# Strong-AI-Lab/ct-vae

Hardware: AMD Instinct MI355X
Metric: images/sec/GPU fwd+bwd, 64×64×3 bs=64; recon+KL vs CPU ref (higher is better)
Workload: dtype f32; 1 GPU; VanillaVAE 64x64x3 train step fwd+loss+bwd+Adam (configs/vae.yaml shapes at the batch BASELINE.json's metric names, bs=64, on one MI355X; BASELINE.json configs[1..4] are the `configs` entries); per_gpu_batch=64, global_batch=64, latent_dim=128, parallelism=single, hipgraph=True, allreduce_overlap=False

## Files before the change

ct-vae_amd/csrc/api.hip:

```cpp
#include "../../include/ctvae_hip.h"

#include "common.hpp"
#include "gatlayer.hpp"
#include "glinear.hpp"
#include "pair.hpp"

namespace ctvae {
int launch_tapgemm(const ConvGeom& g, const float* G, const float* W, const float* bias, const float* add,
                   const float* mask, int mask_act, float* S, int act, float* bn_part, float* ws, size_t ws_floats,
                   hipStream_t st, const BnBwdFuse* bnb = nullptr, const InXform* xf = nullptr,
                   const WinoFilters* wf = nullptr, SplitKRaw* raw = nullptr, int out_pix = 0);
bool out_pix_supported(const ConvGeom& g, size_t ws_floats, int out_pix);
bool wino_supported(const ConvGeom& g, size_t ws_floats);
bool wino_enabled();
int wino_set_enabled(int on);
int launch_crop_resize_u8(const unsigned char* img, const long long* rows, float* out, int B, int N, int H, int W, int crop,
                          int S, hipStream_t st);
bool thin_forward_supported(const ConvGeom& g);
bool thin_wgrad_supported(const ConvGeom& g);
int tapgemm_bnb_rows(const ConvGeom& g, size_t ws_floats);
bool img_dgrad_supported(const ConvGeom& g);
void tapgemm_plan(const ConvGeom& g, size_t ws_floats, TapGemmPlan& p);
int launch_wgrad(const ConvGeom& g, const float* X, const float* dY, float* dW, float* dbias, float* ws, size_t ws_bytes,
                 int accumulate, hipStream_t st, const InXform* xf = nullptr, const DyXform* dyx = nullptr);
int launch_bn_forward(const float* y, int R, int C, const float* gamma, const float* beta, float* running_mean,
                      float* running_var, float momentum, float eps, int training, int act, float* out, float* save_mean,
                      float* save_invstd, float* ws, size_t ws_bytes, long long* nbt, hipStream_t st,
                      float* coef_out = nullptr);
int launch_bn_finish_forward(const float* y, int R, int C, int nparts, const float* gamma, const float* beta,
                             float* running_mean, float* running_var, float momentum, float eps, int training, int act,
                             float* out, float* save_mean, float* save_invstd, float* ws, long long* nbt, hipStream_t st,
                             float* coef_out = nullptr);
size_t bn_workspace_floats(int C, int nparts);
int launch_bn_backward(const float* ga, const float* beta, const float* y, int R, int C, const float* gamma,
                       const float* save_mean, const float* save_invstd, int act, float* gy, float* dgamma, float* dbeta,
                       int accumulate, float* ws, size_t ws_bytes, const float* part_in, int part_rows, hipStream_t st,
                       float* coef_out = nullptr, const float* coef_in = nullptr);
int launch_wino_filters_batch(int n, const float* const* W, float* const* Uf, float* const* Ub, const int* Ci, const int* Co,
                              hipStream_t st);
bool upconv_wgrad_supported(const ConvGeom& g);
bool img_enc_supported(const ConvGeom& g);
bool img_conv_supported(const ConvGeom& g);
int launch_img_backward_fused(const ConvGeom& g, const float* dY, const float* W, float* dX, const BnBwdFuse* bnb, float* ws,
                              float** part_out, float** pbias_out, int* nparts, bool want_bias, hipStream_t st);
size_t img_backward_fused_ws_floats(const ConvGeom& g);
int wgrad_finish_slabs(const float* part, float* dW, long n, int nparts, const float* pbias, float* dbias, long nb, int accumulate,
                       hipStream_t st);
int launch_permute(const float* in, float* out, int B, int C, int P, int to_nhwc, hipStream_t st);
int launch_gat_score(int mode, const float* xl, const float* xr, const float* attr, const float* we, const float* att, float* out,
                     int B, int N, int H, int C, float slope, hipStream_t st);
int launch_gat_score_backward(const float* xl, const float* xr, const float* attr, const float* we, const float* att,
                              const float* g, float* dxl, float* dxr, float* datt_part, float* dwe_part, int B, int N, int H,
                              int C, float slope, hipStream_t st);
int launch_gauss_latent_fwd(float* heads, const float* eps_in, const unsigned long long* rng, float* eps_out, float* z, int B,
                            int L, hipStream_t st, const float* slices, int S, const float* bias);
int launch_splitk_permute(const float* slices, int S, float* out, int B, int C, int P, hipStream_t st);
int launch_gauss_latent_bwd(const float* g_mu, const float* g_lv, const float* g_z, const float* heads, const float* eps,
                            float* g_heads, unsigned long long* rng_bump, int B, int L, hipStream_t st, int gz_slices);
int launch_ct_reg_forward(const float* adj, const float* graph, const float* uni, float* part, float ckl, float cgs, float cpt,
                          int B, int N, hipStream_t st);
int launch_ct_reg_backward(const float* adj, const float* graph, const float* uni, const float* part, const float* g_loss,
                           float ckl, float cgs, float cpt, float* d_adj, float* d_graph, int B, int N, hipStream_t st);
int launch_ct_blend_softmax_forward(const float* y, const float* mask, float* probs, long R, int Hs, int D, hipStream_t st);
int launch_ct_blend_softmax_backward(const float* g, const float* probs, const float* y, const float* mask, float* dy, float* dmask,
                                     long R, int Hs, int D, hipStream_t st);
int launch_ct_latent_ce_forward(const float* probs, const long long* target, float* row_loss, long R, int D, hipStream_t st);
int launch_ct_latent_ce_backward(const float* probs, const long long* target, const float* g_loss, float* d_probs, long R, int D,
                                 hipStream_t st);
int launch_ct_mask_forward(const float* x, const float* action, const float* pe, const float* keep, float scale, const float* W,
                           const float* bias, const float* expo, int B, int S, int D, int A, float* inter, float* p, float* sample,
// ... 440 lines not shown
}

int ctvae_conv_wgrad_bn_apply_supported(int kind, int B, int H, int W, int Ci, int Co, int k, int stride, int pad, int out_pad) {
  if (!conv_kind_ok(kind)) return 0;
  ConvGeom g;
  if (conv_geom(g, kind, 0, B, H, W, Ci, Co, k, stride, pad, out_pad)) return 0;
  if (upconv_wgrad_supported(g)) return 1;
  return img_enc_supported(g) ? 2 : 0;
}

int ctvae_bn_forward(const float* y, int R, int C, const float* gamma, const float* beta, float* running_mean,
                     float* running_var, float momentum, float eps, int training, int act, float* out,
                     float* save_mean, float* save_invstd, int64_t* num_batches_tracked, float* ws, size_t ws_bytes,
                     void* stream) {
  if (!y || !gamma || !beta || !out || !ws) return kErrBadArg;
  if (training && (!save_mean || !save_invstd)) return kErrBadArg;
  if (!training && (!running_mean || !running_var)) return kErrBadArg;
  return launch_bn_forward(y, R, C, gamma, beta, running_mean, running_var, momentum, eps, training, act, out, save_mean,
                           save_invstd, ws, ws_bytes, (long long*)num_batches_tracked, (hipStream_t)stream);
}

int ctvae_bn_backward(const float* g_a, const float* beta, const float* y, int R, int C, const float* gamma,
                      const float* save_mean, const float* save_invstd, int act, float* g_y, float* dgamma,
                      float* dbeta, int accumulate, const float* part_in, int part_rows, float* coef_out,
                      const float* coef_in, float* ws, size_t ws_bytes, void* stream) {
  if (!g_a || !beta || !y || !gamma || !save_mean || !save_invstd || !dgamma || !dbeta || !ws) return kErrBadArg;
  if (!g_y && !coef_out) return kErrBadArg;
  if ((part_in != nullptr) != (part_rows > 0)) return kErrBadArg;
  if (coef_in != nullptr && (!g_y || part_in != nullptr || coef_out != nullptr)) return kErrBadArg;
  return launch_bn_backward(g_a, beta, y, R, C, gamma, save_mean, save_invstd, act, g_y, dgamma, dbeta, accumulate, ws,
                            ws_bytes, part_in, part_rows, (hipStream_t)stream, coef_out, coef_in);
}

int ctvae_gat_score(int mode, const float* xl, const float* xr, const float* attr, const float* we, const float* att, float* out,
                    int B, int N, int H, int C, float slope, void* stream) {
  if (!xl || !xr || !attr || !we || !att || !out || (mode != 0 && mode != 1)) return kErrBadArg;
  return launch_gat_score(mode, xl, xr, attr, we, att, out, B, N, H, C, slope, (hipStream_t)stream);
}

int ctvae_gat_score_backward(const float* xl, const float* xr, const float* attr, const float* we, const float* att,
                             const float* g, float* d_xl, float* d_xr, float* d_att_part, float* d_we_part, int B, int N, int H,
                             int C, float slope, void* stream) {
  if (!xl || !xr || !attr || !we || !att || !g || !d_xl || !d_xr || !d_att_part || !d_we_part) return kErrBadArg;
  return launch_gat_score_backward(xl, xr, attr, we, att, g, d_xl, d_xr, d_att_part, d_we_part, B, N, H, C, slope,
                                   (hipStream_t)stream);
}

int ctvae_gat_layer_forward(const float* xl, const float* xr, int ld, const float* adj, const float* we, const float* att,
                            const float* bias, const int32_t* head_map, float* out, int ldo, float* alpha, int B, int Hs, int C,
                            float slope, int act, void* stream) {
  const GatLayerArgs a{xl, xr, ld, adj, we, att, bias, head_map, out, ldo, alpha, B, Hs, C, slope, act};
  return launch_gat_layer_forward(a, (hipStream_t)stream);
}

int ctvae_gat_layer_backward(const float* xl, const float* xr, int ld, const float* adj, const float* we, const float* att,
                             const float* bias, const int32_t* head_map, const float* out, int ldo, const float* alpha,
                             const float* g_out, float* dS, float* dattr, float* d_xl, float* d_xr, int ldd, float* d_bias_part,
                             float* d_att_part, float* d_we_part, float* d_adj, int accumulate_dadj, int B, int Hs, int C,
                             float slope, int act, void* stream) {
  GatBwdArgs p{};
  p.f = GatLayerArgs{xl, xr, ld, adj, we, att, bias, head_map, const_cast<float*>(out), ldo, const_cast<float*>(alpha), B, Hs, C,
                     slope, act};
  p.g_out = g_out; p.dS = dS; p.dattr = dattr; p.dxl = d_xl; p.dxr = d_xr; p.ldd = ldd;
  p.dbias_part = d_bias_part; p.datt_part = d_att_part; p.dwe_part = d_we_part;
  return launch_gat_layer_backward(p, d_adj, accumulate_dadj, (hipStream_t)stream);
}
// ... 473 lines not shown
```

ct-vae_amd/csrc/bn.hip:

```cpp
#include "common.hpp"
#include "phase.hpp"
#include "finish.hpp"
#include "prof.hpp"

namespace ctvae {
__device__ __forceinline__ float act_dt(float t, int act, float slope) {
  return act == ACT_TANH ? act_bwd_from_out(act_fwd(t, ACT_TANH), ACT_TANH) : act_slope_bwd(t, slope);
}


constexpr int kBnMaxBlocks = 2048;

__device__ __forceinline__ void chan_merge(float& n, float& mean, float& m2, float nb, float mb, float qb) {
  if (nb > 0.f) {
    const float nt = n + nb, d = mb - mean;
    mean += d * (nb / nt);
    m2 += qb + d * d * (n * nb / nt);
    n = nt;
  }
}

__global__ __launch_bounds__(256) void bn_stats_partial_kernel(const float* __restrict__ y, float* __restrict__ part,
                                                               int R, int C, int rows_per_block) {
  __shared__ float sm[256 * 9];
// ... 315 lines not shown
  }
  s1 = wave_sum_d(s1);
  s2 = wave_sum_d(s2);
  if ((tid & 63) == 0) { sm[(tid >> 6) * 2] = s1; sm[(tid >> 6) * 2 + 1] = s2; }
  __syncthreads();
  if (tid == 0) {
    s1 = (sm[0] + sm[2]) + (sm[4] + sm[6]);
    s2 = (sm[1] + sm[3]) + (sm[5] + sm[7]);
    const float db = (float)s1, dg = (float)s2;
    dgamma[c] = (accumulate ? dgamma[c] : 0.f) + dg;
    dbeta[c] = (accumulate ? dbeta[c] : 0.f) + db;
    const float invstd = save_invstd[c], mean = save_mean[c];
    const float k1 = gamma[c] * invstd;
    const float k2 = -k1 * dg / R * invstd;
    const float k3 = -k1 * db / R - k2 * mean;
    coef[c] = k1;
    coef[C + c] = k2;
    coef[2 * C + c] = k3;
    coef[3 * C + c] = k1;
    coef[4 * C + c] = beta[c] - mean * k1;
  }
}

__global__ __launch_bounds__(256) void bn_bwd_finalize_apply_kernel(const float* __restrict__ ga, const float* __restrict__ y,
                                                                    const float* __restrict__ part, int nblocks, int R, int C,
                                                                    const float* __restrict__ gamma, const float* __restrict__ save_mean,
                                                                    const float* __restrict__ save_invstd, const float* __restrict__ beta,
                                                                    int act, float* __restrict__ gy, float* __restrict__ dgamma,
                                                                    float* __restrict__ dbeta, int accumulate) {
  __shared__ double smd[256 * 2];
  __shared__ __attribute__((aligned(16))) float sK[5][32];
  const int tid = threadIdx.x, cb = blockIdx.x, rs = blockIdx.y;
  const int c0 = cb * 32, ch = tid & 31, rl = tid >> 5;
  double s1 = 0.0, s2 = 0.0;
  for (int b = rl; b < nblocks; b += 8) {
    s1 += (double)part[((long)b * C + c0 + ch) * 2 + 0];
    s2 += (double)part[((long)b * C + c0 + ch) * 2 + 1];
  }
  smd[tid * 2] = s1; smd[tid * 2 + 1] = s2;
  __syncthreads();
  if (rl == 0) {
    for (int l = 1; l < 8; ++l) {
      s1 += smd[(l * 32 + ch) * 2];
      s2 += smd[(l * 32 + ch) * 2 + 1];
    }
    const int c = c0 + ch;
    const float db = (float)s1, dg = (float)s2;
    const float invstd = save_invstd[c], mean = save_mean[c];
    const float k1 = gamma[c] * invstd;
    const float k2 = -k1 * dg / (float)R * invstd;
    const float k3 = -k1 * db / (float)R - k2 * mean;
    sK[0][ch] = k1; sK[1][ch] = k2; sK[2][ch] = k3; sK[3][ch] = k1; sK[4][ch] = beta[c] - mean * k1;
    if (rs == 0) {
      dgamma[c] = (accumulate ? dgamma[c] : 0.f) + dg;
      dbeta[c] = (accumulate ? dbeta[c] : 0.f) + db;
    }
  }
  __syncthreads();
  const int q = tid & 7;
  const f32x4 k1 = *reinterpret_cast<const f32x4*>(&sK[0][4 * q]), k2 = *reinterpret_cast<const f32x4*>(&sK[1][4 * q]);
  const f32x4 k3 = *reinterpret_cast<const f32x4*>(&sK[2][4 * q]), sc = *reinterpret_cast<const f32x4*>(&sK[3][4 * q]);
  const f32x4 sh = *reinterpret_cast<const f32x4*>(&sK[4][4 * q]);
  const int rows_per = (R + gridDim.y - 1) / gridDim.y;
  const int r0 = rs * rows_per, r1 = r0 + rows_per < R ? r0 + rows_per : R;
  for (int r = r0 + (tid >> 3); r < r1; r += 32) {
    const long i = ((long)r * C + c0) / 4 + q;
    const f32x4 g = reinterpret_cast<const f32x4*>(ga)[i], yv = reinterpret_cast<const f32x4*>(y)[i];
    f32x4 o;
#pragma unroll
    for (int k = 0; k < 4; ++k)
      o[k] = k1[k] * (g[k] * act_dt(yv[k] * sc[k] + sh[k], act, act_slope(act))) + k2[k] * yv[k] + k3[k];
    reinterpret_cast<f32x4*>(gy)[i] = o;
  }
}

__global__ __launch_bounds__(256) void bn_bwd_finalize_job_kernel(BnFinJob j) {
  __shared__ double sm[8];
  bn_bwd_finalize_body(j, blockIdx.x, sm);
// ... 363 lines not shown
  } else {
    hipLaunchKernelGGL(bn_eval_coeff_kernel, dim3(ceil_div(C, 256)), dim3(256), 0, st, C, gamma, beta, running_mean,
                       running_var, eps, scale, shift);
    CTVAE_LAUNCH_CHECK();
  }
  if (out == nullptr) return 0;
  const long n4 = (long)R * C / 4;
  long blocks = (n4 + 255) / 256;
  if (blocks > 4096) blocks = 4096;
  ProfScope ps("bn_apply_act_kernel", st, 0.0, 8.0 * (double)R * C);
  hipLaunchKernelGGL(bn_apply_act_kernel, dim3((unsigned)blocks), dim3(256), 0, st, y, scale, shift, out, n4, C, act);
  CTVAE_LAUNCH_CHECK();
  return 0;
}

int launch_bn_forward(const float* y, int R, int C, const float* gamma, const float* beta, float* running_mean,
                      float* running_var, float momentum, float eps, int training, int act, float* out,
                      float* save_mean, float* save_invstd, float* ws, size_t ws_bytes, long long* nbt, hipStream_t st,
                      float* coef_out) {
  if (!bn_shape_ok(R, C)) return kErrBadArg;
  if (ws_bytes / sizeof(float) < bn_workspace_floats(C, 0)) return kErrWorkspace;
  int nb = 0;
  if (training) {
    int rpb;
    nb = stat_blocks(R, C, &rpb);
    ProfScope ps("bn_stats_partial_kernel", st, 0.0, 4.0 * (double)R * C);
    hipLaunchKernelGGL(bn_stats_partial_kernel, dim3(nb), dim3(256), 0, st, y, ws, R, C, rpb);
    CTVAE_LAUNCH_CHECK();
  }
  return launch_bn_finish_forward(y, R, C, nb, gamma, beta, running_mean, running_var, momentum, eps, training, act, out,
                                  save_mean, save_invstd, ws, nbt, st, coef_out);
}

int launch_bn_backward(const float* ga, const float* beta, const float* y, int R, int C, const float* gamma,
                       const float* save_mean, const float* save_invstd, int act, float* gy, float* dgamma,
                       float* dbeta, int accumulate, float* ws, size_t ws_bytes, const float* part_in, int part_rows,
                       hipStream_t st, float* coef_out, const float* coef_in) {
  if (!bn_shape_ok(R, C)) return kErrBadArg;
  if (coef_in != nullptr) {
    if (gy == nullptr) return kErrBadArg;
    ProfScope ps("bn_bwd_apply_kernel", st, 0.0, 12.0 * (double)R * C);
    const long n4 = (long)R * C / 4;
    long blocks = (n4 + 255) / 256;
    if (blocks > 4096) blocks = 4096;
    hipLaunchKernelGGL(bn_bwd_apply_kernel, dim3((unsigned)blocks), dim3(256), 0, st, ga, y, coef_in, gy, n4, C, act, dgamma,
                       dbeta, accumulate);
    CTVAE_LAUNCH_CHECK();
    return 0;
  }
  if (ws_bytes / sizeof(float) < bn_workspace_floats(C, 0)) return kErrWorkspace;
  const float* part = ws;
  float* coef = coef_out != nullptr ? coef_out : ws + (size_t)kBnMaxBlocks * C * 3;
  int rpb;
  int nb = stat_blocks(R, C, &rpb);
  if (part_in != nullptr && part_rows > 0) {
    part = part_in;
    nb = part_rows;
  } else {
    ProfScope ps("bn_bwd_partial_kernel", st, 0.0, 8.0 * (double)R * C);
    hipLaunchKernelGGL(bn_bwd_partial_kernel, dim3(nb), dim3(256), 0, st, ga, gamma, beta, y, save_mean, save_invstd, ws, R,
                       C, rpb, act);
  }
  CTVAE_LAUNCH_CHECK();
  if (part_in != nullptr && gy != nullptr && coef_out == nullptr && nb <= 256 && C % 32 == 0) {
    int rsn = 512 / (C / 32);
    if (rsn > R / 32) rsn = R / 32;
    if (rsn < 1) rsn = 1;
    ProfScope ps("bn_bwd_finalize_apply_kernel", st, 0.0, 12.0 * (double)R * C + 8.0 * (double)nb * C * rsn);
    hipLaunchKernelGGL(bn_bwd_finalize_apply_kernel, dim3(C / 32, rsn), dim3(256), 0, st, ga, y, part, nb, R, C, gamma, save_mean,
                       save_invstd, beta, act, gy, dgamma, dbeta, accumulate);
    CTVAE_LAUNCH_CHECK();
    return 0;
  }
  {
    ProfScope ps("bn_bwd_finalize_kernel", st, 0.0, 8.0 * (double)nb * C);
    hipLaunchKernelGGL(bn_bwd_finalize_kernel, dim3(C), dim3(256), 0, st, part, nb, C, (float)R, gamma,
                       save_mean, save_invstd, dgamma, dbeta, accumulate, beta, coef);
  }
  CTVAE_LAUNCH_CHECK();
  if (gy == nullptr) return 0;
  ProfScope ps("bn_bwd_apply_kernel", st, 0.0, 12.0 * (double)R * C);
  const long n4 = (long)R * C / 4;
  long blocks = (n4 + 255) / 256;
  if (blocks > 4096) blocks = 4096;
  hipLaunchKernelGGL(bn_bwd_apply_kernel, dim3((unsigned)blocks), dim3(256), 0, st, ga, y, coef, gy, n4, C, act, (float*)nullptr,
                     (float*)nullptr, 0);
  CTVAE_LAUNCH_CHECK();
  return 0;
}

int launch_bn_bwd_finalize_job(const BnFinJob& j, hipStream_t st) {
  ProfScope ps("bn_bwd_finalize_kernel", st, 0.0, 8.0 * (double)j.nblocks * j.C);
  hipLaunchKernelGGL(bn_bwd_finalize_job_kernel, dim3(j.C), dim3(256), 0, st, j);
  CTVAE_LAUNCH_CHECK();
  return 0;
}

// ... 2 lines not shown
```

ct-vae_amd/kernels.py:

```python
import math
import weakref
from dataclasses import dataclass

import torch
from torch.autograd import Function

from . import native

ACT_NONE, ACT_LRELU, ACT_RELU, ACT_TANH = 0, 1, 2, 3
CONV, CONVT = 0, 1
CONV_FLAT = CONV | 0x100
BN_MOMENTUM, BN_EPS = 0.1, 1e-5


@dataclass(frozen=True)
class ConvSpec:
    kind: int
    ci: int
    co: int
    k: int
    stride: int = 1
    pad: int = 0
    out_pad: int = 0
    act: int = ACT_NONE
# ... 124 lines not shown

def _wino_filters_for(ctx_needs_grad, w, spec, B, H, W_):
    n = wino_filter_floats(spec, B, H, W_, native.workspace(w.device).numel()) if ctx_needs_grad else 0
    if not n:
        return None, None
    if _WINO_BATCH and spec.ci % 32 == 0 and spec.co % 32 == 0:
        uf, ub = wino_cache.filters(w, spec, n)
        return uf, ub
    return None, torch.empty(n, dtype=torch.float32, device=w.device)


def conv_dgrad_raw(dy, w, spec: ConvSpec, in_hw, add=None, mask=None, mask_act=ACT_NONE, wino_filters=None):
    B = dy.shape[0]
    H, W = in_hw
    dx = torch.empty((B, H, W, spec.ci), dtype=torch.float32, device=dy.device)
    ws = native.workspace(dy.device)
    if wino_filters is not None and wino_filter_floats(spec, B, H, W, ws.numel()) != wino_filters.numel():
        wino_filters = None
    g = spec.geom(B, H, W)
    native.call("ctvae_conv_dgrad", g[0], dy.data_ptr(), w.data_ptr(), native.ptr(add), native.ptr(mask), mask_act,
                dx.data_ptr(), *g[1:], native.ptr(wino_filters), ws.data_ptr(), ws.numel() * 4)
    return dx


def _stamp(t):
    return t.data_ptr(), t._version, tuple(t.shape)


def _same(t, stamp):
    return stamp is not None and _stamp(t) == stamp


class BNLink:
    __slots__ = ("y", "mean", "invstd", "gamma", "beta", "act", "part", "rows", "coef", "g", "slices", "sole", "g_hold")

    def __init__(self, y, mean, invstd, gamma, beta, act):
        self.y, self.mean, self.invstd, self.gamma, self.beta, self.act = y, mean, invstd, gamma, beta, act
        self.sole = False
        self.g_hold = None
        self.part = None
        self.rows = 0
        self.coef = None
        self.slices = None
        self.g = None

    def publish_lazy(self, g, slices, n, geom):
        self.slices = (slices, n, geom)
        self.g_hold = g
        self.part, self.rows, self.coef = None, 0, None
        self.g = _stamp(g)

    def take_lazy(self, g):
        sl, self.slices = self.slices, None
        self.g_hold = None
        if sl is None:
            return None
        if not _same(g, self.g):
            raise RuntimeError("BNLink: the consumer left its data gradient as split-K slices for this BatchNorm's backward pass "
                               "(sole consumer of the layer's output), but a different gradient tensor arrived")
        return sl

    def publish(self, g, part, rows, coef=None):
        self.part, self.rows, self.coef = part, rows, coef
        self.g = _stamp(g)

    def take(self, g):
        part, rows, coef = self.part, self.rows, self.coef
        self.part, self.rows, self.coef = None, 0, None
        if part is None or not _same(g, self.g):
            return None, 0, None
        return part, rows, coef
# ... 80 lines not shown


def pop_lazy_bn():
    global _last_lazy
    lz, _last_lazy = _last_lazy, None
    return lz


def bn_apply_is_separate(spec, B, H, W) -> bool:
    ws = native.workspace(torch.device("cuda", torch.cuda.current_device()))
    return bool(_geom_query("ctvae_conv_bn_act_apply_is_separate", spec.geom(B, H, W), ws.numel() * 4))


def lazy_bn_input_supported(spec, B, H, W) -> bool:
    return input_transform_supported(spec, B, H, W)


def pop_bn_link():
    global _last_link
    link, _last_link = _last_link, None
    return link


def mark_sole_consumer(x):
    link = getattr(x, "_ctvae_bn_link", None)
    if link is not None:
        link.sole = True
    return x


def link_of(x):
    link = getattr(x, "_ctvae_bn_link", None)
    return link if (link is not None and x.is_contiguous()) else None


def _dy_bn_args(dy_bn):
    return (dy_bn[0].data_ptr(), dy_bn[1].data_ptr(), dy_bn[2], native.ptr(dy_bn[3])) if dy_bn is not None else (None, None, 0, None)


def _bn_commit_args(bn_commit):
    return (bn_commit[0].data_ptr(), bn_commit[1].data_ptr(), bn_commit[2]) if bn_commit is not None else (None, None, 0)


def conv_wgrad_raw(x, dy, w_param, b_param, spec: ConvSpec, in_coef=None, in_act=ACT_NONE, dy_bn=None, bn_commit=None):
    B, H, W, _ = x.shape
    ws = native.workspace(x.device)
    gw, gb, acc = _grad_targets(w_param, b_param)
    g = spec.geom(B, H, W)
    native.call("ctvae_conv_wgrad", g[0], x.data_ptr(), dy.data_ptr(), gw.data_ptr(), native.ptr(gb), *g[1:], acc,
                *_coef_ptrs(in_coef, spec.ci), in_act, *_dy_bn_args(dy_bn), *_bn_commit_args(bn_commit),
                ws.data_ptr(), ws.numel() * 4)


_PAIR = True


def _conv_backward_lazy(x, dy, w_param, gw, gb, acc, spec, in_coef, in_act, pixel_major):
    B, H, W, _ = x.shape
    ws = native.workspace(x.device)
    g = spec.geom(B, H, W)
    n = _geom_query("ctvae_conv_backward_lazy_slices", g, 0 if pixel_major else 1, ws.numel() * 4)
    if n <= 1:
        return None
    slices = torch.empty(n * B * H * W * spec.ci, dtype=torch.float32, device=dy.device)
    native.call("ctvae_conv_backward_lazy", g[0], x.data_ptr(), dy.data_ptr(), w_param.data_ptr(), gw.data_ptr(), native.ptr(gb),
                slices.data_ptr(), *g[1:], acc, *_coef_ptrs(in_coef, spec.ci), in_act, pixel_major, ws.data_ptr(), ws.numel() * 4)
    return slices, n


def conv_backward_raw(x, dy, w_param, b_param, spec: ConvSpec, link=None, mask=None, mask_act=ACT_NONE, wino_filters=None,
                      in_coef=None, in_act=ACT_NONE, dy_bn=None, bn_commit=None, grad_slices=False):
    B, H, W, _ = x.shape
    ws = native.workspace(x.device)
    g = spec.geom(B, H, W)
    if wino_filters is not None and wino_filter_floats(spec, B, H, W, ws.numel() // 2) != wino_filters.numel():
        wino_filters = None
    gw, gb, acc = _grad_targets(w_param, b_param)
    dx = torch.empty((B, H, W, spec.ci), dtype=torch.float32, device=dy.device)
    if (link is not None and link.sole and tuple(link.y.shape) == (B, H, W, spec.ci) and mask is None and wino_filters is None
            and dy_bn is None and bn_commit is None):
        lazy = _conv_backward_lazy(x, dy, w_param, gw, gb, acc, spec, in_coef, in_act, 0)
        if lazy is not None:
            link.publish_lazy(dx, *lazy, g)
            return dx
    if grad_slices and link is None and mask is None and wino_filters is None and dy_bn is None and bn_commit is None:
        lazy = _conv_backward_lazy(x, dy, w_param, gw, gb, acc, spec, in_coef, in_act, 1)
        if lazy is not None:
            offer_lazy_grad(dx, *lazy)
            return dx
    part, rows = None, 0
    if link is not None and tuple(link.y.shape) == (B, H, W, spec.ci):
        rows = max(_geom_query("ctvae_conv_backward_bn_rows", g, ws.numel() * 4), 0)
        if rows > 0:
            part = torch.empty(rows * spec.ci * 2, dtype=torch.float32, device=dy.device)
    bn = link if part is not None else None
    coef = torch.empty(7 * spec.ci, dtype=torch.float32, device=dy.device) if bn is not None else None
    cg, cb, cacc = _bn_commit_args(bn_commit)
    if coef is None:
        cg = cb = None
    native.call("ctvae_conv_backward", g[0], x.data_ptr(), dy.data_ptr(), w_param.data_ptr(), gw.data_ptr(), native.ptr(gb),
                dx.data_ptr(), *g[1:], acc, native.ptr(mask), mask_act, native.ptr(wino_filters),
                native.ptr(bn.y if bn else None), native.ptr(bn.mean if bn else None), native.ptr(bn.invstd if bn else None),
                native.ptr(bn.gamma if bn else None), native.ptr(bn.beta if bn else None), bn.act if bn else 0,
                native.ptr(part), rows, native.ptr(coef), cg, cb, cacc,
                *_coef_ptrs(in_coef, spec.ci), in_act, *_dy_bn_args(dy_bn), ws.data_ptr(), ws.numel() * 4)
    if bn is not None:
        bn.publish(dx, part, rows, coef)
    return dx


def wgrad_then_dgrad(x, g, w_param, b_param, spec, need_dgrad, link=None, wino_filters=None, in_coef=None, in_act=ACT_NONE,
                     grad_slices=False):
    if need_dgrad:
        return conv_backward_raw(x, g, w_param, b_param, spec, link=link, wino_filters=wino_filters, in_coef=in_coef, in_act=in_act,
                                 grad_slices=grad_slices)
    conv_wgrad_raw(x, g, w_param, b_param, spec, in_coef=in_coef, in_act=in_act)
    return None


def act_backward_raw(g_out, out, act):
    if act == ACT_NONE:
        return g_out
    g_in = torch.empty_like(out)
    native.call("ctvae_act_backward", g_out.data_ptr(), out.data_ptr(), g_in.data_ptr(), out.numel(), act)
    return g_in


def permute_raw(x, B, C, P, to_nhwc):
    out = torch.empty(x.numel(), dtype=torch.float32, device=x.device)
# ... 296 lines not shown
                *_coef_ptrs(in_coef, spec.ci), in_act, ws.data_ptr(), ws.numel() * 4)
    return y, a, coef, save_mean, save_invstd


def _bn_backward(g_a, y, bn, bn_act, g_y, grads, part=None, rows=0, coef_out=None, coef_in=None):
    gamma, beta, save_mean, save_invstd = bn
    gg, gbt, acc = grads
    B, H, W, C = y.shape
    ws = native.workspace(y.device)
    native.call("ctvae_bn_backward", g_a.data_ptr(), beta.data_ptr(), y.data_ptr(), B * H * W, C, gamma.data_ptr(),
                save_mean.data_ptr(), save_invstd.data_ptr(), bn_act, native.ptr(g_y), gg.data_ptr(), gbt.data_ptr(), acc,
                native.ptr(part), rows, native.ptr(coef_out), native.ptr(coef_in), ws.data_ptr(), ws.numel() * 4)


class ConvBNAct(Function):

    @staticmethod
    def forward(ctx, x, w, b, gamma, beta, running_mean, running_var, training, spec, bn_act, num_batches_tracked=None,
                lazy_out=False):
        global _last_link
        _req_cuda(x, w, gamma)
        ctx.link_in = link_of(x)
        ctx.x_slices_ok = bool(getattr(x, "_ctvae_grad_slices_ok", False))
        lazy_in = getattr(x, "_ctvae_lazy_bn", None) if x.is_contiguous() else None
        x = _c(x)
        y, a, coef, save_mean, save_invstd = _conv_bn_act_forward(
            x, (w, b, gamma, beta), (running_mean, running_var, num_batches_tracked), training, spec, bn_act, lazy_in,
            want_a=not lazy_out, want_coef=lazy_out)
        ctx.spec, ctx.bn_act, ctx.training = spec, bn_act, training
        ctx.params = (w, b, gamma, beta)
        ctx.lazy_in = lazy_in
        ctx.save_for_backward(x, y, save_mean, save_invstd)
        ctx.link_out = _last_link = BNLink(y, save_mean, save_invstd, gamma, beta, bn_act) if training else None
        if lazy_out:
            global _last_lazy
            _last_lazy = (coef, bn_act)
            return y
        return a

    @staticmethod
    def backward(ctx, g_a):
        if not ctx.training:
            raise RuntimeError("backward through eval-mode BatchNorm is not supported on the HIP path")
        spec = ctx.spec
        w, b, gamma, beta = ctx.params
        x, y, save_mean, save_invstd = ctx.saved_tensors
        g_a = _c(g_a)
        in_coef, in_act = ctx.lazy_in if ctx.lazy_in is not None else (None, ACT_NONE)
        gg, gbt, accg = _grad_targets(gamma, beta)
        lazy = ctx.link_out.take_lazy(g_a) if ctx.link_out is not None else None
        if lazy is not None:
            g_y = torch.empty_like(y)
            native.call("ctvae_bn_backward_fused", lazy[0].data_ptr(), lazy[1], *lazy[2], y.data_ptr(), gamma.data_ptr(),
                        beta.data_ptr(), save_mean.data_ptr(), save_invstd.data_ptr(), ctx.bn_act, g_y.data_ptr(), gg.data_ptr(),
                        gbt.data_ptr(), accg)
        else:
            part, rows, coef = ctx.link_out.take(g_a) if ctx.link_out is not None else (None, 0, None)
            if coef is not None:
                part, rows = None, 0
                if not ctx.needs_input_grad[0] and wgrad_bn_apply_mode(spec, x.shape[0], x.shape[1], x.shape[2]) == 2:
                    conv_wgrad_raw(x, g_a, w, b, spec, dy_bn=(y, coef, ctx.bn_act, None), bn_commit=(gg, gbt, accg))
                    return (None,) * 12
            g_y = torch.empty_like(y)
            _bn_backward(g_a, y, (gamma, beta, save_mean, save_invstd), ctx.bn_act, g_y, (gg, gbt, accg), part, rows, coef_in=coef)
        g_x = wgrad_then_dgrad(x, g_y, w, b, spec, ctx.needs_input_grad[0], ctx.link_in, in_coef=in_coef, in_act=in_act,
                               grad_slices=ctx.x_slices_ok)
# ... 1385 lines not shown
```

ct-vae_amd/native.py:

```python
import ctypes
import os

import torch

_HERE = os.path.dirname(os.path.abspath(__file__))
LIB_PATH = os.environ.get("CTVAE_LIB_OVERRIDE") or os.path.join(_HERE, "lib", "libctvae_hip.so")

_c = ctypes
_fp, _vp, _i, _l, _f, _sz = _c.c_void_p, _c.c_void_p, _c.c_int, _c.c_long, _c.c_float, _c.c_size_t

SIGNATURES = {
    "ctvae_linear_pixmajor_supported": [_i, _i, _i, _i, _sz],
    "ctvae_linear_pixmajor_forward": [_fp, _fp, _fp, _fp, _i, _i, _i, _i, _i, _fp, _sz, _vp],
    "ctvae_conv_forward": [_i, _fp, _fp, _fp, _fp, _fp] + [_i] * 10 + [_fp, _fp, _i, _fp, _fp, _fp, _sz, _vp],
    "ctvae_wino_filters_batch": [_i, _vp, _vp, _vp, _vp, _vp, _vp],
    "ctvae_conv_bn_act_forward": [_i, _fp, _fp, _fp, _fp, _fp, _fp, _fp, _f, _f, _i, _i, _fp, _fp, _fp, _fp, _fp, _fp] + [_i] * 9
                                 + [_fp, _fp, _i, _fp, _sz, _vp],
    "ctvae_conv_dgrad": [_i, _fp, _fp, _fp, _fp, _i, _fp] + [_i] * 9 + [_fp, _fp, _sz, _vp],
    "ctvae_conv_wgrad": [_i, _fp, _fp, _fp, _fp] + [_i] * 10 + [_fp, _fp, _i, _fp, _fp, _i, _fp, _fp, _fp, _i, _fp, _sz, _vp],
    "ctvae_conv_backward": [_i, _fp, _fp, _fp, _fp, _fp, _fp] + [_i] * 10 + [_fp, _i, _fp, _fp, _fp, _fp, _fp, _fp, _i, _fp, _i,
                            _fp, _fp, _fp, _i, _fp, _fp, _i, _fp, _fp, _i, _fp, _fp, _sz, _vp],
    "ctvae_conv_backward_lazy": [_i, _fp, _fp, _fp, _fp, _fp, _fp] + [_i] * 10 + [_fp, _fp, _i, _i, _fp, _sz, _vp],
    "ctvae_bn_backward_fused": [_fp, _i] + [_i] * 10 + [_fp, _fp, _fp, _fp, _fp, _i, _fp, _fp, _fp, _i, _vp],
    "ctvae_bn_forward": [_fp, _i, _i, _fp, _fp, _fp, _fp, _f, _f, _i, _i, _fp, _fp, _fp, _fp, _fp, _sz, _vp],
# ... 72 lines not shown
    "ctvae_dip_backward": [_fp, _fp, _fp, _fp, _i, _i, _vp],
    "ctvae_column_moments": [_fp, _i, _i, _fp, _fp, _fp, _fp, _vp],
    "ctvae_mi_matrix": [_fp, _fp, _fp, _fp, _fp, _i, _i, _i, _fp, _fp, _vp],
    "ctvae_group_var_argmin": [_fp, _fp, _fp, _i, _i, _i, _fp, _fp, _vp],
    "ctvae_image_grid_u8": [_fp, _l, _l, _l, _l, _i, _i, _i, _i, _i, _i, _i, _i, _f, _f, _f, _i, _fp, _sz, _fp, _sz, _vp],
    "ctvae_adam_step": [_fp, _fp, _fp, _fp, _fp, _l, _f, _vp],
    "ctvae_adam_step_clipped": [_fp, _fp, _fp, _fp, _fp, _l, _f, _i, _f, _fp, _fp, _vp],
    "ctvae_mssim_forward": [_fp, _fp, _fp, _fp, _fp, _fp, _fp, _i, _i, _i, _i, _vp],
    "ctvae_mssim_backward": [_fp, _fp, _fp, _fp, _fp, _fp, _i, _i, _i, _i, _vp],
    "ctvae_defer_begin": [_fp, _sz],
    "ctvae_defer_flush": [_vp],
}
_RESTYPES = {
    "ctvae_version": _c.c_char_p,
    "ctvae_arch": _c.c_char_p,
    "ctvae_error_string": _c.c_char_p,
    "ctvae_workspace_bytes": _c.c_size_t,
    "ctvae_prof_enable": None,
    "ctvae_prof_calibrate": None,
    "ctvae_prof_report": _c.c_size_t,
    "ctvae_conv_backward_bn_rows": _c.c_int,
    "ctvae_conv_backward_lazy_slices": _c.c_int,
    "ctvae_conv_forward_lazy_slices": _c.c_int,
    "ctvae_conv_bn_act_apply_is_separate": _c.c_int,
    "ctvae_winograd_enable": _c.c_int,
    "ctvae_conv_wino_filter_floats": _c.c_size_t,
    "ctvae_dip_state_floats": _c.c_size_t,
    "ctvae_adam_state_floats": _c.c_size_t,
    "ctvae_grad_clip_workspace_floats": _c.c_size_t,
    "ctvae_mssim_part_floats": _c.c_size_t,
    "ctvae_glinear_wgrad_ws_bytes": _c.c_size_t,
    "ctvae_conv_input_transform_supported": _c.c_int,
    "ctvae_conv_wgrad_bn_apply_supported": _c.c_int,
}
EXPORTS = sorted(list(SIGNATURES) + list(_RESTYPES))

_lib = None


def load():
    global _lib
    if _lib is not None:
        return _lib
    if not os.path.exists(LIB_PATH):
        raise RuntimeError(
            f"{LIB_PATH} is missing: build it with `python -m ctvae_amd.build` (hipcc, gfx950). "
            "There is no CPU/PyTorch fallback for the ctvae hot path.")
    try:
        lib = ctypes.CDLL(LIB_PATH)
    except OSError as e:
        raise RuntimeError(f"cannot load {LIB_PATH}: {e}") from e
    for name, argtypes in SIGNATURES.items():
        fn = getattr(lib, name, None)
        if fn is None:
            raise RuntimeError(f"{LIB_PATH} does not export {name} (stale build?)")
        fn.argtypes = argtypes
        fn.restype = _c.c_int
    for name, res in _RESTYPES.items():
        fn = getattr(lib, name, None)
        if fn is None:
            raise RuntimeError(f"{LIB_PATH} does not export {name} (stale build?)")
        fn.restype = res
        fn.argtypes = {"ctvae_error_string": [_c.c_int], "ctvae_prof_enable": [_c.c_int],
                       "ctvae_prof_calibrate": [_c.c_void_p, _c.c_int],
                       "ctvae_prof_report": [_c.c_char_p, _c.c_size_t],
                       "ctvae_conv_backward_bn_rows": [_c.c_int] * 10 + [_c.c_size_t],
                       "ctvae_conv_backward_lazy_slices": [_c.c_int] * 11 + [_c.c_size_t],
                       "ctvae_conv_forward_lazy_slices": [_c.c_int] * 10 + [_c.c_size_t],
                       "ctvae_conv_bn_act_apply_is_separate": [_c.c_int] * 10 + [_c.c_size_t],
                       "ctvae_winograd_enable": [_c.c_int],
                       "ctvae_dip_state_floats": [_c.c_int, _c.c_int],
                       "ctvae_glinear_wgrad_ws_bytes": [_c.c_int, _c.c_int, _c.c_int],
                       "ctvae_conv_wino_filter_floats": [_c.c_int] * 10 + [_c.c_size_t],
                       "ctvae_conv_input_transform_supported": [_c.c_int] * 10,
                       "ctvae_conv_wgrad_bn_apply_supported": [_c.c_int] * 10}.get(name, [])
    if lib.ctvae_arch() != b"gfx950":
        raise RuntimeError("libctvae_hip.so was not built for gfx950")
    _lib = lib
    return lib


def check(code: int, what: str):
    if code != 0:
        msg = load().ctvae_error_string(int(code)).decode()
        raise RuntimeError(f"{what} failed: {msg} (code {code})")


def stream_ptr() -> int:
    return torch.cuda.current_stream().cuda_stream


def ptr(t):
    return None if t is None else t.data_ptr()


_workspaces = {}


def workspace(device) -> torch.Tensor:
    key = (device.index if device.index is not None else torch.cuda.current_device(), torch.cuda.current_stream().cuda_stream)
    ws = _workspaces.get(key)
    if ws is None:
        n = load().ctvae_workspace_bytes()
        ws = torch.empty(n // 4, dtype=torch.float32, device=device)
        _workspaces[key] = ws
    return ws


# ... 42 lines not shown
```

include/ctvae_hip.h:

```cpp
#ifndef CTVAE_HIP_H
#define CTVAE_HIP_H
#include <stddef.h>
#include <stdint.h>

#ifdef __cplusplus
extern "C" {
#endif

#define CTVAE_ACT_NONE 0
#define CTVAE_ACT_LRELU 1
#define CTVAE_ACT_RELU 2
#define CTVAE_ACT_TANH 3

#define CTVAE_CONV 0
#define CTVAE_CONVT 1
#define CTVAE_W_CI_TAP 0x100

const char* ctvae_version(void);
const char* ctvae_arch(void);
const char* ctvae_error_string(int code);
size_t ctvae_workspace_bytes(void);

int ctvae_conv_forward(int kind, const float* x, const float* w, const float* bias, const float* add, float* y, int B,
                       int H, int W, int Ci, int Co, int k, int stride, int pad, int out_pad, int act, const float* in_scale,
// ... 29 lines not shown
                     void* stream);
int ctvae_conv_backward_bn_rows(int kind, int B, int H, int W, int Ci, int Co, int k, int stride, int pad, int out_pad,
                                size_t ws_bytes);
int ctvae_conv_backward(int kind, const float* x, const float* dy, const float* w, float* dw, float* dbias, float* dx, int B,
                        int H, int W, int Ci, int Co, int k, int stride, int pad, int out_pad, int accumulate, const float* mask,
                        int mask_act, const float* wino_filters, const float* bn_y, const float* bn_mean,
                        const float* bn_invstd, const float* bn_gamma, const float* bn_beta, int bn_act, float* bn_part,
                        int bn_part_rows, float* bn_coef_out, float* bn_dgamma, float* bn_dbeta, int bn_accumulate,
                        const float* in_scale, const float* in_shift, int in_act,
                        const float* dy_bn_y, const float* dy_bn_coef, int dy_bn_act, float* gy_out, float* ws, size_t ws_bytes,
                        void* stream);

int ctvae_conv_backward_lazy_slices(int kind, int B, int H, int W, int Ci, int Co, int k, int stride, int pad, int out_pad,
                                    int for_bn, size_t ws_bytes);
int ctvae_conv_backward_lazy(int kind, const float* x, const float* dy, const float* w, float* dw, float* dbias, float* dx_slices,
                             int B, int H, int W, int Ci, int Co, int k, int stride, int pad, int out_pad, int accumulate,
                             const float* in_scale, const float* in_shift, int in_act, int pixel_major, float* ws, size_t ws_bytes,
                             void* stream);
int ctvae_bn_backward_fused(const float* g_a_slices, int slices, int kind, int B, int H, int W, int Ci, int Co, int k, int stride,
                            int pad, int out_pad, const float* y, const float* gamma, const float* beta, const float* save_mean,
                            const float* save_invstd, int act, float* g_y, float* dgamma, float* dbeta, int accumulate, void* stream);

int ctvae_conv_wgrad_bn_apply_supported(int kind, int B, int H, int W, int Ci, int Co, int k, int stride, int pad,
                                        int out_pad);

int ctvae_bn_forward(const float* y, int R, int C, const float* gamma, const float* beta, float* running_mean,
                     float* running_var, float momentum, float eps, int training, int act, float* out,
                     float* save_mean, float* save_invstd, int64_t* num_batches_tracked, float* ws, size_t ws_bytes,
                     void* stream);
int ctvae_bn_backward(const float* g_a, const float* beta, const float* y, int R, int C, const float* gamma,
                      const float* save_mean, const float* save_invstd, int act, float* g_y, float* dgamma,
                      float* dbeta, int accumulate, const float* part_in, int part_rows, float* coef_out,
                      const float* coef_in, float* ws, size_t ws_bytes, void* stream);

int ctvae_pair_mlp_forward(const float* u, const float* v, int ld, const float* w2, const float* b2, float* out, int B, int N,
                           int H, float slope, int per_sample, const int32_t* row_of, void* stream);
int ctvae_pair_mlp_backward(const float* u, const float* v, int ld, const float* w2, const float* out, const float* g_out,
                            float* d_u, float* d_v, int ldd, float* d_w2_part, float* d_b2_part, int B, int N, int H, float slope,
                            int per_sample, const int32_t* row_of, void* stream);

int ctvae_gat_score(int mode, const float* xl, const float* xr, const float* attr, const float* we, const float* att, float* out,
                    int B, int N, int H, int C, float slope, void* stream);
int ctvae_gat_score_backward(const float* xl, const float* xr, const float* attr, const float* we, const float* att,
                             const float* g, float* d_xl, float* d_xr, float* d_att_part, float* d_we_part, int B, int N, int H,
                             int C, float slope, void* stream);

int ctvae_gat_layer_forward(const float* xl, const float* xr, int ld, const float* adj, const float* we, const float* att,
                            const float* bias, const int32_t* head_map, float* out, int ldo, float* alpha, int B, int Hs, int C,
                            float slope, int act, void* stream);
int ctvae_gat_layer_backward(const float* xl, const float* xr, int ld, const float* adj, const float* we, const float* att,
                             const float* bias, const int32_t* head_map, const float* out, int ldo, const float* alpha,
                             const float* g_out, float* dS, float* dattr, float* d_xl, float* d_xr, int ldd, float* d_bias_part,
                             float* d_att_part, float* d_we_part, float* d_adj, int accumulate_dadj, int B, int Hs, int C,
                             float slope, int act, void* stream);

int ctvae_glinear_forward(const float* x, int ldx, int K, int nseg, int N, const float* const* W, const int* ldw,
                          const int64_t* w_gstride, const float* const* bias, const int* b_gstride,
                          const int32_t* const* group, float* y, int ldy, int B, void* stream);
int ctvae_glinear_dgrad(const float* dy, int ldy, int nseg, int N, const float* const* W, const int* ldw,
                        const int64_t* w_gstride, const int32_t* const* group, float* dx, int ldx, int K, int B, void* stream);
size_t ctvae_glinear_wgrad_ws_bytes(int G, int N, int K);
int ctvae_glinear_wgrad(const float* x, int ldx, int K, const float* dy, int ldy, int col0, int N, const int32_t* group, int G,
                        int B, float* dW, int ldo, float* dbias, int accumulate, float* ws, size_t ws_bytes, void* stream);

int ctvae_ct_blend_forward(const float* s0, const float* s1, const float* mask, float* out, long rows, void* stream);
int ctvae_ct_blend_backward(const float* g, const float* s0, const float* s1, const float* mask, float* g0, float* g1, float* g_mask,
// ... 174 lines not shown
```

Measured before the change: 89060 images/s.

## Use one-launch BN backward when apply follows and widen partial reduction

The BN backward partial-sum reduction now loads 32 partial rows per thread with vector loads and tree-reduces them in registers, instead of a strided serial loop. The Python side now skips allocating and producing a separate coefficient buffer when a BN apply step follows and the one-launch path is supported, so BN backward runs in a single fused kernel rather than a coefficient pass plus an apply. This adds register pressure (64 doubles per thread) and routes more layers through the fused path.

Measured after the change: 88280 images/s. Within noise of the previous version (-0.9%).

```diff
diff --git a/ct-vae_amd/csrc/api.hip b/ct-vae_amd/csrc/api.hip
--- a/ct-vae_amd/csrc/api.hip
+++ b/ct-vae_amd/csrc/api.hip
@@ -36,6 +36,7 @@
                        const float* save_mean, const float* save_invstd, int act, float* gy, float* dgamma, float* dbeta,
                        int accumulate, float* ws, size_t ws_bytes, const float* part_in, int part_rows, hipStream_t st,
                        float* coef_out = nullptr, const float* coef_in = nullptr);
+bool bn_bwd_one_launch(int nb, int C);
 int launch_wino_filters_batch(int n, const float* const* W, float* const* Uf, float* const* Ub, const int* Ci, const int* Co,
                               hipStream_t st);
 bool upconv_wgrad_supported(const ConvGeom& g);
@@ -542,6 +543,8 @@
                             ws_bytes, part_in, part_rows, (hipStream_t)stream, coef_out, coef_in);
 }
 
+int ctvae_bn_backward_one_launch(int part_rows, int C) { return bn_bwd_one_launch(part_rows, C) ? 1 : 0; }
+
 int ctvae_gat_score(int mode, const float* xl, const float* xr, const float* attr, const float* we, const float* att, float* out,
                     int B, int N, int H, int C, float slope, void* stream) {
   if (!xl || !xr || !attr || !we || !att || !out || (mode != 0 && mode != 1)) return kErrBadArg;
diff --git a/ct-vae_amd/csrc/bn.hip b/ct-vae_amd/csrc/bn.hip
--- a/ct-vae_amd/csrc/bn.hip
+++ b/ct-vae_amd/csrc/bn.hip
@@ -371,18 +371,35 @@
   __shared__ __attribute__((aligned(16))) float sK[5][32];
   const int tid = threadIdx.x, cb = blockIdx.x, rs = blockIdx.y;
   const int c0 = cb * 32, ch = tid & 31, rl = tid >> 5;
-  double s1 = 0.0, s2 = 0.0;
-  for (int b = rl; b < nblocks; b += 8) {
-    s1 += (double)part[((long)b * C + c0 + ch) * 2 + 0];
-    s2 += (double)part[((long)b * C + c0 + ch) * 2 + 1];
-  }
+  double a1[32], a2[32];
+#pragma unroll
+  for (int u = 0; u < 32; ++u) a1[u] = a2[u] = 0.0;
+  for (int base = 0; base < nblocks; base += 256) {
+    f32x2 t[32];
+#pragma unroll
+    for (int u = 0; u < 32; ++u) {
+      const int b = base + 32 * rl + u;
+      t[u] = *reinterpret_cast<const f32x2*>(part + ((long)(b < nblocks ? b : 0) * C + c0 + ch) * 2);
+    }
+#pragma unroll
+    for (int u = 0; u < 32; ++u) {
+      if (base + 32 * rl + u < nblocks) { a1[u] += (double)t[u][0]; a2[u] += (double)t[u][1]; }
+    }
+  }
+#pragma unroll
+  for (int w = 1; w < 32; w *= 2) {
+#pragma unroll
+    for (int u = 0; u < 32; u += 2 * w) { a1[u] += a1[u + w]; a2[u] += a2[u + w]; }
+  }
+  double s1 = a1[0], s2 = a2[0];
   smd[tid * 2] = s1; smd[tid * 2 + 1] = s2;
   __syncthreads();
   if (rl == 0) {
-    for (int l = 1; l < 8; ++l) {
-      s1 += smd[(l * 32 + ch) * 2];
-      s2 += smd[(l * 32 + ch) * 2 + 1];
-    }
+    double p1[8], p2[8];
+#pragma unroll
+    for (int l = 0; l < 8; ++l) { p1[l] = smd[(l * 32 + ch) * 2]; p2[l] = smd[(l * 32 + ch) * 2 + 1]; }
+    s1 = ((p1[0] + p1[1]) + (p1[2] + p1[3])) + ((p1[4] + p1[5]) + (p1[6] + p1[7]));
+    s2 = ((p2[0] + p2[1]) + (p2[2] + p2[3])) + ((p2[4] + p2[5]) + (p2[6] + p2[7]));
     const int c = c0 + ch;
     const float db = (float)s1, dg = (float)s2;
     const float invstd = save_invstd[c], mean = save_mean[c];
@@ -812,6 +829,8 @@
                                   save_mean, save_invstd, ws, nbt, st, coef_out);
 }
 
+bool bn_bwd_one_launch(int nb, int C) { return nb > 0 && nb <= 256 && C % 32 == 0; }
+
 int launch_bn_backward(const float* ga, const float* beta, const float* y, int R, int C, const float* gamma,
                        const float* save_mean, const float* save_invstd, int act, float* gy, float* dgamma,
                        float* dbeta, int accumulate, float* ws, size_t ws_bytes, const float* part_in, int part_rows,
@@ -842,7 +861,7 @@
                        C, rpb, act);
   }
   CTVAE_LAUNCH_CHECK();
-  if (part_in != nullptr && gy != nullptr && coef_out == nullptr && nb <= 256 && C % 32 == 0) {
+  if (part_in != nullptr && gy != nullptr && coef_out == nullptr && bn_bwd_one_launch(nb, C)) {
     int rsn = 512 / (C / 32);
     if (rsn > R / 32) rsn = R / 32;
     if (rsn < 1) rsn = 1;
diff --git a/ct-vae_amd/kernels.py b/ct-vae_amd/kernels.py
--- a/ct-vae_amd/kernels.py
+++ b/ct-vae_amd/kernels.py
@@ -180,11 +180,13 @@
 
 
 class BNLink:
-    __slots__ = ("y", "mean", "invstd", "gamma", "beta", "act", "part", "rows", "coef", "g", "slices", "sole", "g_hold")
+    __slots__ = ("y", "mean", "invstd", "gamma", "beta", "act", "part", "rows", "coef", "g", "slices", "sole", "g_hold",
+                 "apply_follows")
 
     def __init__(self, y, mean, invstd, gamma, beta, act):
         self.y, self.mean, self.invstd, self.gamma, self.beta, self.act = y, mean, invstd, gamma, beta, act
         self.sole = False
+        self.apply_follows = False
         self.g_hold = None
         self.part = None
         self.rows = 0
@@ -331,6 +333,10 @@
 def link_of(x):
     link = getattr(x, "_ctvae_bn_link", None)
     return link if (link is not None and x.is_contiguous()) else None
+
+
+def bn_backward_one_launch(rows, C) -> bool:
+    return bool(native.load().ctvae_bn_backward_one_launch(rows, C))
 
 
 def _dy_bn_args(dy_bn):
@@ -393,7 +399,8 @@
         if rows > 0:
             part = torch.empty(rows * spec.ci * 2, dtype=torch.float32, device=dy.device)
     bn = link if part is not None else None
-    coef = torch.empty(7 * spec.ci, dtype=torch.float32, device=dy.device) if bn is not None else None
+    own = bn is not None and bn.apply_follows and bn_commit is None and bn_backward_one_launch(rows, spec.ci)
+    coef = torch.empty(7 * spec.ci, dtype=torch.float32, device=dy.device) if bn is not None and not own else None
     cg, cb, cacc = _bn_commit_args(bn_commit)
     if coef is None:
         cg = cb = None
@@ -756,6 +763,9 @@
         ctx.lazy_in = lazy_in
         ctx.save_for_backward(x, y, save_mean, save_invstd)
         ctx.link_out = _last_link = BNLink(y, save_mean, save_invstd, gamma, beta, bn_act) if training else None
+        if training:
+            ctx.link_out.apply_follows = (ctx.needs_input_grad[0] or
+                                          wgrad_bn_apply_mode(spec, x.shape[0], x.shape[1], x.shape[2]) != 2)
         if lazy_out:
             global _last_lazy
             _last_lazy = (coef, bn_act)
diff --git a/ct-vae_amd/native.py b/ct-vae_amd/native.py
--- a/ct-vae_amd/native.py
+++ b/ct-vae_amd/native.py
@@ -128,6 +128,7 @@
     "ctvae_glinear_wgrad_ws_bytes": _c.c_size_t,
     "ctvae_conv_input_transform_supported": _c.c_int,
     "ctvae_conv_wgrad_bn_apply_supported": _c.c_int,
+    "ctvae_bn_backward_one_launch": _c.c_int,
 }
 EXPORTS = sorted(list(SIGNATURES) + list(_RESTYPES))
 
@@ -169,7 +170,8 @@
                        "ctvae_glinear_wgrad_ws_bytes": [_c.c_int, _c.c_int, _c.c_int],
                        "ctvae_conv_wino_filter_floats": [_c.c_int] * 10 + [_c.c_size_t],
                        "ctvae_conv_input_transform_supported": [_c.c_int] * 10,
-                       "ctvae_conv_wgrad_bn_apply_supported": [_c.c_int] * 10}.get(name, [])
+                       "ctvae_conv_wgrad_bn_apply_supported": [_c.c_int] * 10,
+                       "ctvae_bn_backward_one_launch": [_c.c_int, _c.c_int]}.get(name, [])
     if lib.ctvae_arch() != b"gfx950":
         raise RuntimeError("libctvae_hip.so was not built for gfx950")
     _lib = lib
diff --git a/include/ctvae_hip.h b/include/ctvae_hip.h
--- a/include/ctvae_hip.h
+++ b/include/ctvae_hip.h
@@ -85,6 +85,7 @@
                       const float* save_mean, const float* save_invstd, int act, float* g_y, float* dgamma,
                       float* dbeta, int accumulate, const float* part_in, int part_rows, float* coef_out,
                       const float* coef_in, float* ws, size_t ws_bytes, void* stream);
+int ctvae_bn_backward_one_launch(int part_rows, int C);
 
 int ctvae_pair_mlp_forward(const float* u, const float* v, int ld, const float* w2, const float* b2, float* out, int B, int N,
                            int H, float slope, int per_sample, const int32_t* row_of, void* stream);
```
